# ROAM-Lab-ND/generalized_rbda

Measured on AMD Instinct MI355X. Metric: forward-dynamics evals/sec (batched random states), MIT Humanoid cluster model, higher is better.
Workload: dtype f32; 1 GPU; mit_humanoid.urdf cluster-ABA, 262144 random states per GPU; batch_per_gpu=262144, batch_global=262144, nq=25, nv=24, n_bodies=37, n_clusters=17, parallelism=batch-sharded x1, plan replicated

## Files before the change

### generalized_rbda_amd/csrc/capi.cpp

```cpp
#include <hip/hip_runtime.h>

#include <array>
#include <cassert>
#include <cmath>
#include <cstdio>
#include <cstdlib>
#include <cstring>
#include <map>
#include <memory>
#include <mutex>
#include <string>
#include <vector>

#include "../../include/grbda_hip.h"
#include "../../include/grbda_hip_vjp.h"
#include "../../include/grbda_model_desc.h"
#include "devplan.h"

namespace grbda_hip {
int urdf_to_blob(const char *const *paths, int n_paths, int ori_repr, std::vector<unsigned char> &blob,
                 std::string &err);

}

// ... 2471 lines not shown
        size_t B, int device, void *stream)
{
    if (!p) return set_err(GRBDA_EINVAL, "null plan");
    GRBDA_CALL_SCOPE(p);
    if (int rc = vjp_args<T>(p, q, qd, x, g, step, grad_q, grad_qd, grad_x, ydd_out, B)) return rc;
    if (B == 0) return GRBDA_OK;
    return vjp_run<T>(p, forward, q, qd, x, g, step, grad_q, grad_qd, grad_x, ydd_out, B, device, stream);
}
int vjp_host_f64(const grbda_plan *p, bool forward, const double *q, const double *qd, const double *x, const double *g, double step, double *grad_q,
                 double *grad_qd, double *grad_x, double *ydd_out, size_t B, int device)
{
    if (!p) return set_err(GRBDA_EINVAL, "null plan");
    GRBDA_CALL_SCOPE(p);
    if (int rc = vjp_args<double>(p, q, qd, x, g, step, grad_q, grad_qd, grad_x, ydd_out, B)) return rc;
    if (B == 0) return GRBDA_OK;
    const size_t nq = p->host.nq, nv = p->host.nv;
    DeviceTables *t = nullptr;
    if (int rc0 = ensure_device(p, device, &t)) return rc0;
    HostStage st;
    const double *bq = st.in(q, B * nq), *bqd = st.in(qd, B * nv), *bx = st.in(x, B * nv), *bg = st.in(g, B * nv);
    double *b1 = grad_q ? st.out(grad_q, B * nv) : nullptr, *b2 = grad_qd ? st.out(grad_qd, B * nv) : nullptr,
           *b3 = grad_x ? st.out(grad_x, B * nv) : nullptr, *b4 = ydd_out ? st.out(ydd_out, B * nv) : nullptr;
    return st.run([&] { return vjp_run<double>(p, forward, bq, bqd, bx, bg, step, b1, b2, b3, b4, B, device, nullptr); });
}

template <class T>
static std::string kernel_name_of(const grbda_plan *p, int kind, int n_cu, size_t B)
{
    const HostPlan &h = p->host;
    const char *tn = sizeof(T) == 4 ? "float" : "double";
    const char *alg = kind == 0 ? "aba" : "rnea";
    const Route r = kind == 0 ? choose_aba<T>(p, n_cu, B, false) : choose_rnea<T>(p, n_cu, B, false);
    char buf[160];
    const auto format = [&](const auto &cp, int gen1_waves) {
        const int segs = !cp.gens.empty() ? 2 : (!cp.diffs.empty() ? 1 : 0);
        if (r.path == ROUTE_GEN1)
            std::snprintf(buf, sizeof buf, "grbda_hip::%s_gen1_kernel<%s, %d, %s, %d>", alg, tn, cp.gens[0].n, cp.gens[0].kind ? "true" : "false", gen1_waves);
        else if (r.path == ROUTE_LM)
            std::snprintf(buf, sizeof buf, "grbda_hip::%s_chain_lm_kernel<%s, %d%s>", alg, tn, r.lm_waves, cp.diffs.empty() ? "" : ", true");
        else if (kind == 0)
            std::snprintf(buf, sizeof buf, "grbda_hip::aba_chain_kernel<%s, %d, %d>", tn, (sizeof(T) == 8 && !cp.gens.empty()) ? 1 : 2, segs);
        else
            std::snprintf(buf, sizeof buf, "grbda_hip::rnea_chain_kernel<%s, %d, %s>", tn, segs, cp.n_glb > 0 ? "true" : "false");
    };
    if (r.path == ROUTE_INTERPRETER) {
        bool loop = false;
        for (const ClusterRec &cr : h.lay64.clusters) loop = loop || cr.kind == CK_LOOP;
        std::snprintf(buf, sizeof buf, "grbda_hip::%s_kernel<%s, %s>", alg, tn, loop ? "true" : "false");
    } else if (kind == 0) {
        format(h.chain[r.slot], r.path == ROUTE_GEN1 ? gen1_waves_per_simd<T>(h.chain[r.slot].gens[0].n) : 0);
    } else {
        const RneaChainProgram &rp = h.rchain[r.slot == SLOT_F32_WIDE ? SLOT_F32 : r.slot];
        format(rp, r.path == ROUTE_GEN1 ? rnea_gen1_waves_per_simd<T>(rp.gens[0].n) : 0);
    }
    return buf;
}

template <class T>
int run_sharded(const grbda_plan *p, bool rnea, const T *q, const T *qd, const T *x, T *out, size_t B, int n_gpus)
{
    if (!p) return set_err(GRBDA_EINVAL, "null plan");
    GRBDA_CALL_SCOPE(p);
    if (!q || !qd || !x || !out) return set_err(GRBDA_EINVAL, "null argument");
    int count = 0;
    if (hipGetDeviceCount(&count) != hipSuccess || count <= 0)
        return set_err(GRBDA_ENODEVICE, "no HIP device available (there is no CPU fallback)");
    if (n_gpus < 1 || n_gpus > count) return set_err(GRBDA_EINVAL, "n_gpus out of range");
    if (B == 0) return GRBDA_OK;
    const size_t nq = p->host.nq, nv = p->host.nv;
    struct Shard {
        size_t b0 = 0, nb = 0;
        T *dq = nullptr, *dqd = nullptr, *dx = nullptr, *dout = nullptr;
        hipStream_t s = nullptr;
    };
    std::vector<Shard> sh(n_gpus);
    int rc = GRBDA_OK;
    hipError_t e = hipSuccess;
    for (int g = 0; g < n_gpus && rc == GRBDA_OK; g++) {
        Shard &S = sh[g];
        S.b0 = B * g / n_gpus;
        S.nb = B * (g + 1) / n_gpus - S.b0;
        if (S.nb == 0) continue;
        if ((e = hipSetDevice(g)) != hipSuccess || (e = hipStreamCreate(&S.s)) != hipSuccess ||
// ... 1106 lines not shown
```

### generalized_rbda_amd/csrc/chain_kernels.hip

```cpp
#include <hip/hip_runtime.h>

#include "devplan.h"

#ifndef GRBDA_CHAIN_UNIT
#define GRBDA_CHAIN_UNIT 0
#endif
#define GRBDA_KLDS (GRBDA_CHAIN_UNIT == 3)

namespace grbda_hip {

#include "devmath.h"

template <class T>
struct ChainTables {
    cptr<ChainSeg> segs;
    cptr<ChainLink> links;
    cptr<ChainPair> pairs;
    cptr<ChainFree> frees;
    cptr<ChainDiff> diffs;
    cptr<ChainGen> gens;
    cptr<ChainGenBody> gbodies;
    cptr<int32_t> cints;
    cptr<T> consts;
    int n_segs, nq, nv, ori_repr;
// ... 75 lines not shown
    {
        return *reinterpret_cast<const T *>(reinterpret_cast<const char *>(base_u + (size_t)(unsigned)(j * kWave)) + (size_t)lane_b);
    }
    __device__ __forceinline__ T q(int j) const { return row_ld(in_q_u, j); }
    __device__ __forceinline__ T qd(int j) const { return row_ld(in_qd_u, j); }
    __device__ __forceinline__ T x(int j) const { return row_ld(in_x_u, j); }
    int out_row;
    __device__ __forceinline__ T got(int j) const
    {
        return *reinterpret_cast<const T *>(reinterpret_cast<const char *>(out_u + (size_t)(unsigned)(j * kWave)) + (size_t)lane_b);
    }
    __device__ __forceinline__ void put_f(int j, T v) const
    {
        if constexpr (sizeof(T) == 4) {
            if (out_row >= 0) reinterpret_cast<T *>(grbda_smem)[(out_row + j) * kWave + lane] = v;
            else put(j, v);
        } else {
            out_f[j * kWave + lane] = v;
        }
    }
    T *out_f;
    __device__ __forceinline__ void set_out(int row)
    {
        out_row = row;
        out_f = row >= 0 ? reinterpret_cast<T *>(grbda_smem) + row * kWave : out_u;
    }
    __device__ __forceinline__ void put(int j, T v) const
    {
        *reinterpret_cast<T *>(reinterpret_cast<char *>(out_u + (size_t)(unsigned)(j * kWave)) + (size_t)lane_b) = v;
    }
};

template <class T>
__device__ __forceinline__ void vxz(const T (&v)[6], T qd, T (&c)[6])
{
    c[0] = v[1] * qd; c[1] = -v[0] * qd; c[2] = 0;
    c[3] = v[4] * qd; c[4] = -v[3] * qd; c[5] = 0;
}

template <class T, class I21>
__device__ __forceinline__ void bias_force(const I21 &I, const T (&v)[6], T (&p)[6])
{
    T Iv[6];
    symv_c(I, v, Iv);
    crf(v, Iv, p);
}

template <class T>
__device__ __forceinline__ void rotor_terms(cptr<T> Rp, const T (&vp)[6], T qdr, T (&tp)[6])
{
    T f[6], t[6];
#pragma unroll
    for (int j = 0; j < 6; j++) f[j] = Rp[j];
    crf(vp, f, t);
#pragma unroll
    for (int j = 0; j < 6; j++) tp[j] = qdr * t[j];
}
template <class T>
__device__ __forceinline__ void rotor_quad(cptr<T> Q, const T (&vp)[6], T (&tp)[6])
{
    T t[6];
    bias_force(Q, vp, t);
#pragma unroll
    for (int j = 0; j < 6; j++) tp[j] += t[j];
}

// ... 50 lines not shown
{
    if (perm < 0) {
        T E[9];
        rotate_z(s, c, C, E);
        xmotion(E, C + 9, vp, v);
        xmotion(E, C + 9, ap, a);
    } else if (perm == 0) {
        xmotion_p<T, 0>(s, c, C + 9, vp, v);
        xmotion_p<T, 0>(s, c, C + 9, ap, a);
    } else if (perm == 1) {
        xmotion_p<T, 1>(s, c, C + 9, vp, v);
        xmotion_p<T, 1>(s, c, C + 9, ap, a);
    } else {
        xmotion_p<T, 2>(s, c, C + 9, vp, v);
        xmotion_p<T, 2>(s, c, C + 9, ap, a);
    }
}
template <class T>
__device__ __forceinline__ void link_force_up(int perm, T s, T c, cptr<T> C, const T (&f)[6], T (&o)[6])
{
    if (perm < 0) {
        T E[9];
        rotate_z(s, c, C, E);
        xforce_inv(E, C + 9, f, o);
    } else if (perm == 0) {
        xforce_inv_p<T, 0>(s, c, C + 9, f, o);
    } else if (perm == 1) {
        xforce_inv_p<T, 1>(s, c, C + 9, f, o);
    } else {
        xforce_inv_p<T, 2>(s, c, C + 9, f, o);
    }
}

template <class T, bool SVG>
__device__ __forceinline__ void run_fwd(const ChainTables<T> &P, const ChainMem<T> &M, const ChainSeg &sg)
{
    T vp[6];
    {
        const ChainLink l0 = load_rec(P.links + sg.first);
        if (l0.lds_pv != -1) {
            if constexpr (SVG) M.acc_ld(l0.lds_pv, vp);
            else M.lds_ld(l0.lds_pv, vp);
        } else {
#pragma unroll
            for (int j = 0; j < 6; j++) vp[j] = 0;
        }
    }
    ChainLink l = load_rec(P.links + sg.first);
    T qi = M.q(l.q_index), qdi_in = M.qd(l.v_index);
    for (int i = 0; i < sg.count; i++) {
        const bool more = i + 1 < sg.count;
        const ChainLink ln = load_rec(P.links + (sg.first + (more ? i + 1 : i)));
        T qn = 0, qdn = 0;
        if (more) {
            qn = M.q(ln.q_index);
            qdn = M.qd(ln.v_index);
        }
        cptr<T> C = P.consts + l.cofs;
        const T g0 = C[kBodyConstFixed];
        T blk[8], v[6];
        const T ang = g0 * qi;
        sincos_t(ang, &blk[0], &blk[1]);
        link_down(perm_if<T>(kPermLink, l.perm), blk[0], blk[1], C, vp, v);
        v[2] += g0 * qdi_in;
#pragma unroll
        for (int j = 0; j < 6; j++) {
            blk[2 + j] = v[j];
            vp[j] = v[j];
        }
        if constexpr (SVG) M.acc_st(l.lds_sv, blk);
        else M.lds_st(l.lds_sv, blk);
        l = ln;
        qi = qn;
        qdi_in = qdn;
    }
}

constexpr int kChunk = 4;
template <class T>
__device__ __forceinline__ void run_fwd_c(const ChainTables<T> &P, const ChainMem<T> &M, const ChainSeg &sg)
{
    T vp[6];
    for (int base = 0; base < sg.count; base += kChunk) {
        const int n = sg.count - base;
        ChainLink L[kChunk];
        T qv[kChunk], qdv[kChunk];
#pragma unroll
        for (int u = 0; u < kChunk; u++) L[u] = load_rec(P.links + (sg.first + base + (u < n ? u : n - 1)));
#pragma unroll
        for (int u = 0; u < kChunk; u++) {
            qv[u] = M.q(L[u].q_index);
            qdv[u] = M.qd(L[u].v_index);
        }
        if (base == 0) {
            if (L[0].lds_pv != -1) {
                M.lds_ld(L[0].lds_pv, vp);
            } else {
#pragma unroll
                for (int j = 0; j < 6; j++) vp[j] = 0;
            }
        }
        T E[kChunk][9], r[kChunk][3], sc[kChunk][2], gq[kChunk];
#pragma unroll
        for (int u = 0; u < kChunk; u++) {
            if (u < n) {
                cptr<T> C = P.consts + L[u].cofs;
                const T g0 = C[kBodyConstFixed];
                sincos_t(g0 * qv[u], &sc[u][0], &sc[u][1]);
                rotate_z(sc[u][0], sc[u][1], C, E[u]);
#pragma unroll
                for (int j = 0; j < 3; j++) r[u][j] = C[9 + j];
                gq[u] = g0 * qdv[u];
            }
// ... 6 lines not shown
                v[2] += gq[u];
                blk[0] = sc[u][0];
                blk[1] = sc[u][1];
#pragma unroll
                for (int j = 0; j < 6; j++) {
                    blk[2 + j] = v[j];
                    vp[j] = v[j];
                }
                M.lds_st(L[u].lds_sv, blk);
            }
        }
    }
}

template <class T, int K>
__device__ __forceinline__ void xmotion_k(T s, T c, const T (&E)[9], cptr<T> C, const T (&m)[6], T (&o)[6])
{
    if constexpr (K < 0) xmotion(E, C + 9, m, o);
    else xmotion_p<T, K>(s, c, C + 9, m, o);
}
template <class T, int K>
__device__ __forceinline__ void xforce_inv_k(T s, T c, const T (&E)[9], cptr<T> C, const T (&f)[6], T (&o)[6])
{
    if constexpr (K < 0) xforce_inv(E, C + 9, f, o);
    else xforce_inv_p<T, K>(s, c, C + 9, f, o);
}
template <class T, int K, class A21>
__device__ __forceinline__ void congruence_k(T s, T c, const T (&E)[9], cptr<T> C, const A21 &A, T (&B)[21])
{
    if constexpr (K < 0) congruence(E, C + 9, A, B);
    else congruence_p<T, K>(s, c, C + 9, A, B);
}

template <class T, bool OSIM, int K1, int K2>
__device__ __forceinline__ void pair_bwd_k(const ChainTables<T> &P, const ChainMem<T> &M, const ChainPair &pr, T (&IA)[21],
                                           T (&psi)[6])
{
    cptr<T> C1 = P.consts + pr.cofs[0], C2 = P.consts + pr.cofs[1];
    T vp[6];
    M.acc_ld(pr.lds_pv, vp);
    const T y1 = M.q(pr.q_index), y2 = M.q(pr.q_index + 1);
    const T yd1 = M.qd(pr.v_index), yd2 = M.qd(pr.v_index + 1);
    T u[2] = {M.x(pr.v_index), M.x(pr.v_index + 1)};
    T D00 = 0, D01 = 0, D11 = 0;
    T F0[6], F1[6];

    T s1, c1, s2, c2, E1[9], E2[9], v1[6], v2[6], ch1[6], ch2[6];
    sincos_t(y1, &s1, &c1);
    if constexpr (K1 < 0) rotate_z(s1, c1, C1, E1);
    xmotion_k<T, K1>(s1, c1, E1, C1, vp, v1);
    v1[2] += yd1;
    vxz(v1, yd1, ch1);
    sincos_t(y2, &s2, &c2);
    if constexpr (K2 < 0) rotate_z(s2, c2, C2, E2);
    xmotion_k<T, K2>(s2, c2, E2, C2, v1, v2);
    v2[2] += yd2;
    vxz(v2, yd2, ch2);
    T ccl2[6];
    xmotion_k<T, K2>(s2, c2, E2, C2, ch1, ccl2);
#pragma unroll
    for (int j = 0; j < 6; j++) ccl2[j] += ch2[j];

    T IA1[21], psi1[6];
    {
        cptr<T> I2 = C2 + 12;
        T p2[6], h2[6];
        bias_force(I2, v2, p2);
#pragma unroll
// ... 48 lines not shown
        D11 += Rp[6] * gb * gb;
#pragma unroll
        for (int j = 0; j < 6; j++) {
            F0[j] += Rp[j] * ga;
            F1[j] += Rp[j] * gb;
            psi[j] += tp[j];
        }
    }
    const T r00 = rsqrt_t(D00), l10 = D01 * r00, r11 = rsqrt_t(D11 - l10 * l10);
    M.pivot(D00);
    M.pivot(D11 - l10 * l10);
    const T i00 = r00 * r00 + (l10 * r00 * r11) * (l10 * r00 * r11), i01 = -(l10 * r00) * r11 * r11, i11 = r11 * r11;
    T blk[14];
    auto solve2 = [&](T b0, T b1, T &x0, T &x1) {
        const T y0 = b0 * r00, y1 = (b1 - l10 * y0) * r11;
        x1 = y1 * r11;
        x0 = (y0 - l10 * x1) * r00;
    };
#pragma unroll
    for (int j = 0; j < 6; j++) solve2(F0[j], F1[j], blk[j], blk[6 + j]);
    solve2(u[0], u[1], blk[12], blk[13]);
    M.glb_st(pr.glb_k, blk);
    if constexpr (OSIM) {
        const T ex[7] = {i00, i01, i11, s1, c1, s2, c2};
        M.glb_st(pr.glb_k + 14, ex);
    }
#pragma unroll
    for (int r = 0; r < 6; r++) {
        psi[r] += F0[r] * blk[12] + F1[r] * blk[13];
#pragma unroll
        for (int cc = r; cc < 6; cc++) IA[sidx(r, cc)] -= F0[r] * blk[cc] + F1[r] * blk[6 + cc];
    }
}
template <class T, bool OSIM>
__device__ __forceinline__ void pair_bwd(const ChainTables<T> &P, const ChainMem<T> &M, const ChainPair &pr, T (&IA)[21],
                                         T (&psi)[6])
{
    if (perm_if<T>(kPermPair, pr.perm[0]) == 0 && pr.perm[1] == 0) pair_bwd_k<T, OSIM, 0, 0>(P, M, pr, IA, psi);
    else pair_bwd_k<T, OSIM, -1, -1>(P, M, pr, IA, psi);
}

template <class T>
__device__ __forceinline__ void pair_acc(const ChainTables<T> &P, const ChainMem<T> &M, const ChainPair &pr)
{
    T blk[14], va[12];
    M.glb_ld(pr.glb_k, blk);
    M.lds_ld(pr.lds_pva, va);
    T y0 = blk[12], y1 = blk[13];
#pragma unroll
    for (int j = 0; j < 6; j++) {
        y0 -= blk[j] * va[6 + j];
        y1 -= blk[6 + j] * va[6 + j];
    }
    M.put_f(pr.v_index, y0);
    M.put_f(pr.v_index + 1, y1);
}


template <class T, class TB>
__device__ __forceinline__ void diff_constraint(const TB &P, const ChainMem<T> &M, int tofs_i, int lds_w, const T (&qs)[4], T yd0,
                                                T yd1, T (&X)[4], T (&g)[2], T (&qdl)[2])
{
    cptr<int32_t> ip = P.cints + tofs_i;
    const int n_args = ip[0], n_atoms = ip[1];
    cptr<T> dp = P.consts + ip[2];
    for (int i = 0; i < n_args; i++) {
        cptr<T> w = dp + 5 * i;
        const T a = w[4] + w[0] * qs[0] + w[1] * qs[1] + w[2] * qs[2] + w[3] * qs[3];
// ... 349 lines not shown
        ydd0 -= blk[j] * ap[j];
        ydd1 -= blk[6 + j] * ap[j];
    }
    M.put_f(d.v_index, ydd0);
    M.put_f(d.v_index + 1, ydd1);
    if (d.lds_va >= 0) {
        cptr<T> C1 = P.consts + d.cofs[0], C2 = P.consts + d.cofs[1];
        const T yd0 = M.qd(d.v_index), yd1 = M.qd(d.v_index + 1);
        const T qd1 = blk[14] * yd0 + blk[15] * yd1, qd2 = blk[16] * yd0 + blk[17] * yd1;
        const T qdd1 = blk[14] * ydd0 + blk[15] * ydd1 + blk[18], qdd2 = blk[16] * ydd0 + blk[17] * ydd1 + blk[19];
        T E1[9], E2[9], v1[6], v2[6], a1[6], a2[6], c[6];
        const T sc[4] = {blk[20], blk[21], blk[22], blk[23]};
        diff_links(C1, C2, sc, vp, qd1, qd2, E1, E2, v1, v2);
        xmotion(E1, C1 + 9, ap, a1);
        vxz(v1, qd1, c);
#pragma unroll
        for (int j = 0; j < 6; j++) a1[j] += c[j];
        a1[2] += qdd1;
        xmotion(E2, C2 + 9, a1, a2);
        vxz(v2, qd2, c);
#pragma unroll
        for (int j = 0; j < 6; j++) a2[j] += c[j];
        a2[2] += qdd2;
        T out[12];
#pragma unroll
        for (int j = 0; j < 6; j++) {
            out[j] = v2[j];
            out[6 + j] = a2[j];
        }
        M.lds_st(d.lds_va, out);
    }
}

template <class T, bool OSIM, bool SVG, int ROT = 0>
__device__ __forceinline__ void run_bwd(const ChainTables<T> &P, const ChainMem<T> &M, const ChainSeg &sg)
{
    T IAc[21], psic[6];
    if (sg.head == HEAD_PAIR) {
        const ChainPair pr = load_rec(P.pairs + sg.head_arg);
        pair_bwd<T, OSIM>(P, M, pr, IAc, psic);
    } else if (sg.head == HEAD_SLOT) {
        T acc[27];
        M.acc_ld(sg.head_arg, acc);
#pragma unroll
        for (int j = 0; j < 21; j++) IAc[j] = acc[j];
#pragma unroll
        for (int j = 0; j < 6; j++) psic[j] = acc[21 + j];
    } else {
#pragma unroll
        for (int j = 0; j < 21; j++) IAc[j] = 0;
#pragma unroll
        for (int j = 0; j < 6; j++) psic[j] = 0;
    }
    ChainLink l = load_rec(P.links + sg.first);
    T yd = M.qd(l.v_index), tau_in = M.x(l.v_index), y_in = M.q(l.q_index);
    T blk[8];
    if constexpr (SVG) M.acc_ld(l.lds_sv, blk);
    for (int i = 0; i < sg.count; i++) {
        const bool more = i + 1 < sg.count;
        const ChainLink ln = load_rec(P.links + (sg.first + (more ? i + 1 : i)));
        T ydn = 0, taun = 0, yn = 0;
        if (more) {
            ydn = M.qd(ln.v_index);
            taun = M.x(ln.v_index);
            yn = M.q(ln.q_index);
        }
        T blkn[8];
        if constexpr (SVG) {
// ... 185 lines not shown
            T v[6], a[6], chat[6], sn, cs;
            sincos_t(g0 * yq, &sn, &cs);
            link_down2(perm_if<T>(kPermAcc, l.perm), sn, cs, C, vp, ap, v, a);
            v[2] += qdi;
            vxz(v, qdi, chat);
#pragma unroll
            for (int j = 0; j < 6; j++) a[j] += chat[j];
            a[2] += g0 * ydd;
            if (l.lds_va >= 0) {
                T va[12];
#pragma unroll
                for (int j = 0; j < 6; j++) {
                    va[j] = v[j];
                    va[6 + j] = a[j];
                }
                M.lds_st(l.lds_va, va);
            }
#pragma unroll
            for (int j = 0; j < 6; j++) {
                vp[j] = v[j];
                ap[j] = a[j];
            }
        }
        if (more) {
            l = ln;
            yd = ydn;
            yq = yqn;
#pragma unroll
            for (int j = 0; j < 7; j++) kb[j] = kn[j];
        }
    }
}

template <class T>
__device__ __forceinline__ void run_acc_c(const ChainTables<T> &P, const ChainMem<T> &M, const ChainSeg &sg)
{
    T vp[6], ap[6];
    for (int base = 0; base < sg.count; base += kChunk) {
        const int n = sg.count - base;
        ChainLink L[kChunk];
        T kb[kChunk][7], yd[kChunk], yq[kChunk];
#pragma unroll
        for (int u = 0; u < kChunk; u++) L[u] = load_rec(P.links + (sg.first + base + (u < n ? u : n - 1)));
#pragma unroll
        for (int u = 0; u < kChunk; u++) {
            yd[u] = M.qd(L[u].v_index);
            yq[u] = M.q(L[u].q_index);
        }
#pragma unroll
        for (int u = 0; u < kChunk; u++) M.glb_ld(L[u].glb_k, kb[u]);
        if (base == 0) {
            if (sg.lds_pva >= 0) {
                T va[12];
                M.lds_ld(sg.lds_pva, va);
#pragma unroll
                for (int j = 0; j < 6; j++) {
                    vp[j] = va[j];
                    ap[j] = va[6 + j];
                }
            } else {
#pragma unroll
                for (int j = 0; j < 6; j++) {
                    vp[j] = 0;
                    ap[j] = P.a_root[j];
                }
            }
        }
        T E[kChunk][9], r[kChunk][3], g0v[kChunk], qdi[kChunk];
// ... 18 lines not shown
                T ydd = kb[u][6];
#pragma unroll
                for (int rr = 0; rr < 6; rr++) ydd -= kb[u][rr] * ap[rr];
                M.put_f(l.v_index, ydd);
                if (l.has_child) {
                    T v[6], a[6], chat[6];
                    xmotion(E[u], r[u], vp, v);
                    xmotion(E[u], r[u], ap, a);
                    v[2] += qdi[u];
                    vxz(v, qdi[u], chat);
#pragma unroll
                    for (int j = 0; j < 6; j++) a[j] += chat[j];
                    a[2] += g0v[u] * ydd;
                    if (l.lds_va >= 0) {
                        T va[12];
#pragma unroll
                        for (int j = 0; j < 6; j++) {
                            va[j] = v[j];
                            va[6 + j] = a[j];
                        }
                        M.lds_st(l.lds_va, va);
                    }
#pragma unroll
                    for (int j = 0; j < 6; j++) {
                        vp[j] = v[j];
                        ap[j] = a[j];
                    }
                }
            }
        }
    }
}

template <class T>
__device__ __forceinline__ void free_fwd(const ChainTables<T> &P, const ChainMem<T> &M, const ChainFree &f)
{
    if (f.lds_v < 0) return;
    T v[6];
#pragma unroll
    for (int j = 0; j < 6; j++) v[j] = M.qd(f.v_index + j);
    M.lds_st(f.lds_v, v);
}

template <class T>
__device__ __forceinline__ void free_acc_inputs(const ChainTables<T> &P, const ChainMem<T> &M, const ChainFree &f, T (&o)[4], T (&r)[3]);
template <class T>
__device__ __forceinline__ void free_acc_core(const ChainTables<T> &P, const ChainMem<T> &M, const ChainFree &f, const T (&y0)[6],
                                              const T (&o)[4], const T (&r)[3], const T (&vb)[6]);
template <class T, bool OSIM>
__device__ __forceinline__ void free_bwd(const ChainTables<T> &P, const ChainMem<T> &M, const ChainFree &f, bool fuse_acc = false)
{
    cptr<T> Ic = P.consts + f.bofs;
    cptr<T> Ib = P.consts + f.iofs;
    T v[6], psi[6], IA[21];
#pragma unroll
    for (int j = 0; j < 6; j++) v[j] = M.qd(f.v_index + j);
    T o_[4] = {0, 0, 0, 0}, r_[3] = {0, 0, 0};
    if constexpr (!OSIM) {
        if (fuse_acc) free_acc_inputs(P, M, f, o_, r_);
    }
    bias_force(Ic, v, psi);
    if (f.lds_acc != -1) {
        T acc[27];
        M.acc_ld(f.lds_acc, acc);
#pragma unroll
        for (int j = 0; j < 21; j++) IA[j] = Ib[j] + acc[j];
#pragma unroll
        for (int j = 0; j < 6; j++) psi[j] += acc[21 + j];
        if (f.lds_acc2 != -1) {
            auto add = [&](int slot) {
                M.acc_ld(slot, acc);
#pragma unroll
                for (int j = 0; j < 21; j++) IA[j] += acc[j];
#pragma unroll
                for (int j = 0; j < 6; j++) psi[j] += acc[21 + j];
            };
            add(f.lds_acc2);
            if (f.lds_acc3 != -1) {
                add(f.lds_acc3);
                if (f.lds_acc4 != -1) add(f.lds_acc4);
            }
        }
    } else {
// ... 1 lines not shown
        for (int j = 0; j < 21; j++) IA[j] = Ib[j];
    }
    T D[6][6], u[6];
#pragma unroll
    for (int i = 0; i < 6; i++) {
        u[i] = M.x(f.v_index + i) - psi[i];
#pragma unroll
        for (int j = 0; j < 6; j++) D[i][j] = IA[sidx(i, j)];
    }
    Chol<T, 6> ch;
    ch.factor(D);
#pragma unroll
    for (int i = 0; i < 6; i++) M.pivot(ch.inv[i] < T(1e30) ? ch.inv[i] : T(0));
    ch.solve(u);
    if constexpr (!OSIM) {
        if (fuse_acc) {
            free_acc_core(P, M, f, u, o_, r_, v);
            return;
        }
    }
    M.glb_st(f.glb_y0, u);
    if constexpr (OSIM) {
        T ex[27];
#pragma unroll
        for (int i = 0; i < 6; i++) {
#pragma unroll
            for (int j = 0; j <= i; j++) ex[i * (i + 1) / 2 + j] = ch.L[i][j];
            ex[21 + i] = ch.inv[i];
        }
        M.glb_st(f.glb_y0 + 6, ex);
    }
}

template <class T>
__device__ __forceinline__ void free_acc_inputs(const ChainTables<T> &P, const ChainMem<T> &M, const ChainFree &f, T (&o)[4], T (&r)[3])
{
    const int nori = P.ori_repr == 0 ? 4 : 3;
#pragma unroll
    for (int j = 0; j < 4; j++) o[j] = j < nori ? M.q(f.q_index + 3 + j) : T(0);
#pragma unroll
    for (int j = 0; j < 3; j++) r[j] = M.q(f.q_index + j);
}
template <class T>
__device__ __forceinline__ void free_acc_core(const ChainTables<T> &P, const ChainMem<T> &M, const ChainFree &f, const T (&y0)[6],
                                              const T (&o)[4], const T (&r)[3], const T (&vb)[6])
{
    T E[9], g[6], ag[6];
    free_rotation(P.ori_repr, o, E);
#pragma unroll
    for (int j = 0; j < 6; j++) g[j] = P.a_root[j];
    xmotion(E, r, g, ag);
#pragma unroll
    for (int j = 0; j < 6; j++) M.put_f(f.v_index + j, y0[j] - ag[j]);
    if (f.lds_va >= 0) {
        T va[12];
#pragma unroll
        for (int j = 0; j < 6; j++) {
            va[j] = vb[j];
            va[6 + j] = y0[j];
        }
        M.lds_st(f.lds_va, va);
    }
}
template <class T>
__device__ __forceinline__ void free_acc(const ChainTables<T> &P, const ChainMem<T> &M, const ChainFree &f)
{
    T y0[6], o[4], r[3], vb[6];
    M.glb_ld(f.glb_y0, y0);
    free_acc_inputs(P, M, f, o, r);
#pragma unroll
    for (int j = 0; j < 6; j++) vb[j] = M.qd(f.v_index + j);
    free_acc_core(P, M, f, y0, o, r, vb);
}

#include "gen_segments.h"

#if GRBDA_CHAIN_UNIT == 2
template <class T>
struct ChainMemC : ChainMem<T> {
    int in_q, in_qd, in_x;
    T *out_g;
    __device__ __forceinline__ T q(int j) const { return reinterpret_cast<const T *>(grbda_smem)[(in_q + j) * kWave + this->lane]; }
    __device__ __forceinline__ T qd(int j) const { return reinterpret_cast<const T *>(grbda_smem)[(in_qd + j) * kWave + this->lane]; }
    __device__ __forceinline__ T x(int j) const { return reinterpret_cast<const T *>(grbda_smem)[(in_x + j) * kWave + this->lane]; }
    __device__ __forceinline__ void put(int j, T v) const
    {
        if (out_g) out_g[j] = v;
    }
    __device__ __forceinline__ void put_f(int j, T v) const { put(j, v); }
};

template <class T, int N, bool LOOP, class BODY>
__device__ __forceinline__ void gen1_tiles(int work_bytes, int nq, const T *__restrict__ q, const T *__restrict__ qd, const T *__restrict__ x,
                                           T *__restrict__ out, size_t B, unsigned long long *bad_count, BODY body)
{
    const int lane = threadIdx.x;
    ChainMemC<T> M;
    M.bad = 0;
// ... 83 lines not shown
template <class T>
int gen1_waves_per_simd(int n)
{
    return sizeof(T) == 4 ? (n <= 2 ? 3 : 2) : (n == 1 ? 2 : 1);
}
template int gen1_waves_per_simd<float>(int);
template int gen1_waves_per_simd<double>(int);
template <class T>
hipError_t launch_aba_gen1(const ChainDev<T> &P, int n, int implicit, const T *q, const T *qd, const T *tau, T *ydd, size_t B, int grid,
                           size_t lds_bytes, hipStream_t stream)
{
    if (implicit) {
        if (n == 1) return launch_gen1<T, 1, true>(P, q, qd, tau, ydd, B, grid, lds_bytes, stream);
        if (n == 2) return launch_gen1<T, 2, true>(P, q, qd, tau, ydd, B, grid, lds_bytes, stream);
        if (n == 3) return launch_gen1<T, 3, true>(P, q, qd, tau, ydd, B, grid, lds_bytes, stream);
        return launch_gen1<T, 4, true>(P, q, qd, tau, ydd, B, grid, lds_bytes, stream);
    }
    if (n == 1) return launch_gen1<T, 1, false>(P, q, qd, tau, ydd, B, grid, lds_bytes, stream);
    if (n == 2) return launch_gen1<T, 2, false>(P, q, qd, tau, ydd, B, grid, lds_bytes, stream);
    if (n == 3) return launch_gen1<T, 3, false>(P, q, qd, tau, ydd, B, grid, lds_bytes, stream);
    return launch_gen1<T, 4, false>(P, q, qd, tau, ydd, B, grid, lds_bytes, stream);
}
template hipError_t launch_aba_gen1<float>(const ChainDev<float> &, int, int, const float *, const float *, const float *, float *, size_t, int,
                                           size_t, hipStream_t);
template hipError_t launch_aba_gen1<double>(const ChainDev<double> &, int, int, const double *, const double *, const double *, double *,
                                            size_t, int, size_t, hipStream_t);
#endif

template <class T, int WPS, int MODE>
__global__ __launch_bounds__(kWave, WPS) void aba_chain_kernel(ChainDev<T> DP, const T *__restrict__ q, const T *__restrict__ qd,
                                                             const T *__restrict__ tau, T *__restrict__ ydd, size_t B,
                                                             T *__restrict__ scratch)
{
    constexpr bool DIFF = MODE >= 1, GEN = MODE == 2;
    ChainTables<T> P;
    P.segs = (cptr<ChainSeg>)DP.segs;
    P.links = (cptr<ChainLink>)DP.links;
    P.pairs = (cptr<ChainPair>)DP.pairs;
    P.frees = (cptr<ChainFree>)DP.frees;
    P.diffs = DIFF ? (cptr<ChainDiff>)DP.diffs : nullptr;
    P.gens = GEN ? (cptr<ChainGen>)DP.gens : nullptr;
    P.gbodies = GEN ? (cptr<ChainGenBody>)DP.gbodies : nullptr;
    P.cints = DIFF ? (cptr<int32_t>)DP.cints : nullptr;
    P.consts = (cptr<T>)DP.consts;
    P.n_segs = DP.n_segs;
    P.nq = DP.nq;
    P.nv = DP.nv;
    P.ori_repr = DP.ori_repr;
#pragma unroll
    for (int i = 0; i < 6; i++) P.a_root[i] = DP.a_root[i];
    const int lane = threadIdx.x;
    T *slab = scratch + (size_t)blockIdx.x * (size_t)(DP.n_glb_slots + P.nq + 2 * P.nv) * kWave;
    ChainMem<T> M;
    M.lane = lane;
    M.lane_b = (unsigned)lane * (unsigned)sizeof(T);
    M.gmul = 1;
    M.amask = ~0;
    M.glb_u = slab + (size_t)(P.nq + 2 * P.nv) * kWave;
    M.in_q_u = slab;
    M.in_qd_u = slab + (size_t)P.nq * kWave;
    M.in_x_u = slab + (size_t)(P.nq + P.nv) * kWave;
    M.out_u = slab + (size_t)(P.nq + P.nv) * kWave;
    M.set_out(DP.out_lds);
    M.bad = 0;

    const size_t n_tiles = (B + kWave - 1) / kWave;
    for (size_t tile = blockIdx.x; tile < n_tiles; tile += gridDim.x) {
        const size_t left = B - tile * kWave;
        const int rows_valid = left < (size_t)kWave ? (int)left : kWave;
        stage_inputs(q, qd, tau, tile, rows_valid, P.nq, P.nv, slab, lane, DP.lds_bytes);
        if (DP.fuse & 1) {
            const T *mine = reinterpret_cast<const T *>(grbda_smem) + (kWave * P.nq + lane * P.nv + DP.stage_v_index);
            T v[6];
#pragma unroll
            for (int j = 0; j < 6; j++) v[j] = mine[j];
            wave_lds_fence();
            M.lds_st(DP.stage_lds_v, v);
        }
        for (int s = 0; s < P.n_segs; s++) {
            const ChainSeg sg = load_rec(P.segs + s);
            switch (sg.op) {
                case SEG_RUN_FWD:
                    if (DP.sv_global) run_fwd<T, true>(P, M, sg);
                    else run_fwd_c(P, M, sg);
                    break;
                case SEG_RUN_BWD: {
                    if (DP.sv_global) run_bwd<T, false, true>(P, M, sg);
                    else if (sg.rot_kind == 1) run_bwd<T, false, false, 1>(P, M, sg);
                    else run_bwd<T, false, false>(P, M, sg);
                    break;
                }
                case SEG_RUN_ACC:
                    run_acc_c(P, M, sg);
                    break;
                case SEG_PAIR_ACC: pair_acc(P, M, load_rec(P.pairs + sg.first)); break;
                case SEG_FREE_FWD:
                    if (!((DP.fuse & 1) && s == 0)) free_fwd(P, M, load_rec(P.frees + sg.first));
                    break;
                case SEG_FREE_BWD: free_bwd<T, false>(P, M, load_rec(P.frees + sg.first), (DP.fuse & 2) != 0); break;
                case SEG_DIFF_FWD:
                    if constexpr (DIFF) diff_fwd(P, M, load_rec(P.diffs + sg.first));
                    break;
                case SEG_DIFF_BWD:
// ... 553 lines not shown
        asm volatile("s_waitcnt vmcnt(0)" ::: "memory");
    }
}

template <class T>
hipError_t launch_osim_chain(const ChainDev<T> &P, const OsimArgs<T> &A, const T *q, const T *zeros, T *Linv, T *J, size_t B,
                             T *scratch, int grid, size_t lds_bytes, hipStream_t stream)
{
    hipLaunchKernelGGL((osim_chain_kernel<T>), dim3(grid), dim3(kWave), lds_bytes, stream, P, A, q, zeros, Linv, J, B, scratch);
    return hipGetLastError();
}
#if GRBDA_CHAIN_UNIT == 0
template hipError_t launch_osim_chain<float>(const ChainDev<float> &, const OsimArgs<float> &, const float *, const float *, float *,
                                             float *, size_t, float *, int, size_t, hipStream_t);
template hipError_t launch_osim_chain<double>(const ChainDev<double> &, const OsimArgs<double> &, const double *, const double *,
                                              double *, double *, size_t, double *, int, size_t, hipStream_t);
#endif

hipError_t launch_aba_chain_diff_f64(const ChainDev<double> &P, const double *q, const double *qd, const double *tau, double *ydd, size_t B,
                                     double *scratch, int grid, size_t lds_bytes, hipStream_t stream);
template <class T>
hipError_t launch_aba_chain_gen(const ChainDev<T> &P, const T *q, const T *qd, const T *tau, T *ydd, size_t B, T *scratch, int grid,
                                size_t lds_bytes, hipStream_t stream);
template <class T>
hipError_t launch_aba_chain(const ChainDev<T> &P, const T *q, const T *qd, const T *tau, T *ydd, size_t B, T *scratch, int grid,
                            size_t lds_bytes, hipStream_t stream)
{
    if (P.n_gens > 0) return launch_aba_chain_gen<T>(P, q, qd, tau, ydd, B, scratch, grid, lds_bytes, stream);
    if (P.n_diffs > 0) {
        if constexpr (sizeof(T) == 8) {
            return launch_aba_chain_diff_f64(P, q, qd, tau, ydd, B, scratch, grid, lds_bytes, stream);
        } else {
            hipLaunchKernelGGL((aba_chain_kernel<T, 2, 1>), dim3(grid), dim3(kWave), lds_bytes, stream, P, q, qd, tau, ydd, B, scratch);
            return hipGetLastError();
        }
    }
    hipLaunchKernelGGL((aba_chain_kernel<T, 2, 0>), dim3(grid), dim3(kWave), lds_bytes, stream, P, q, qd, tau, ydd, B, scratch);
    return hipGetLastError();
}
#if GRBDA_CHAIN_UNIT == 0
template hipError_t launch_aba_chain<float>(const ChainDev<float> &, const float *, const float *, const float *, float *, size_t,
                                            float *, int, size_t, hipStream_t);
template hipError_t launch_aba_chain<double>(const ChainDev<double> &, const double *, const double *, const double *, double *,
                                             size_t, double *, int, size_t, hipStream_t);
#elif GRBDA_CHAIN_UNIT == 1
hipError_t launch_aba_chain_diff_f64(const ChainDev<double> &P, const double *q, const double *qd, const double *tau, double *ydd, size_t B,
                                     double *scratch, int grid, size_t lds_bytes, hipStream_t stream)
{
    hipLaunchKernelGGL((aba_chain_kernel<double, 2, 1>), dim3(grid), dim3(kWave), lds_bytes, stream, P, q, qd, tau, ydd, B, scratch);
    return hipGetLastError();
}
#elif GRBDA_CHAIN_UNIT == 2
template <class T>
hipError_t launch_aba_chain_gen(const ChainDev<T> &P, const T *q, const T *qd, const T *tau, T *ydd, size_t B, T *scratch, int grid,
                                size_t lds_bytes, hipStream_t stream)
{
    if constexpr (sizeof(T) == 8)
        hipLaunchKernelGGL((aba_chain_kernel<T, 1, 2>), dim3(grid), dim3(kWave), lds_bytes, stream, P, q, qd, tau, ydd, B, scratch);
    else
        hipLaunchKernelGGL((aba_chain_kernel<T, 2, 2>), dim3(grid), dim3(kWave), lds_bytes, stream, P, q, qd, tau, ydd, B, scratch);
    return hipGetLastError();
}
template hipError_t launch_aba_chain_gen<float>(const ChainDev<float> &, const float *, const float *, const float *, float *, size_t,
                                                float *, int, size_t, hipStream_t);
template hipError_t launch_aba_chain_gen<double>(const ChainDev<double> &, const double *, const double *, const double *, double *,
                                                 size_t, double *, int, size_t, hipStream_t);
// ... 671 lines not shown
{
    const bool glb = P.n_glb_slots > 0;
    if (P.n_gens > 0) return launch_rnea_chain_gen<T>(P, q, qd, ydd, tau, B, scratch, grid, lds_bytes, stream);
    if (P.n_diffs > 0 && glb) hipLaunchKernelGGL((rnea_chain_kernel<T, 1, true>), dim3(grid), dim3(kWave), lds_bytes, stream, P, q, qd, ydd, tau, B, scratch);
    else if (P.n_diffs > 0) hipLaunchKernelGGL((rnea_chain_kernel<T, 1, false>), dim3(grid), dim3(kWave), lds_bytes, stream, P, q, qd, ydd, tau, B, scratch);
    else if (glb) hipLaunchKernelGGL((rnea_chain_kernel<T, 0, true>), dim3(grid), dim3(kWave), lds_bytes, stream, P, q, qd, ydd, tau, B, scratch);
    else hipLaunchKernelGGL((rnea_chain_kernel<T, 0, false>), dim3(grid), dim3(kWave), lds_bytes, stream, P, q, qd, ydd, tau, B, scratch);
    return hipGetLastError();
}
#if GRBDA_CHAIN_UNIT == 0
template hipError_t launch_rnea_chain<float>(const RneaChainDev<float> &, const float *, const float *, const float *, float *, size_t,
                                             float *, int, size_t, hipStream_t);
template hipError_t launch_rnea_chain<double>(const RneaChainDev<double> &, const double *, const double *, const double *, double *,
                                              size_t, double *, int, size_t, hipStream_t);
#endif


static hipError_t set_max_dynamic_lds(const void *const *kernels, int n)
{
    for (int i = 0; i < n; i++) {
        const hipError_t e = hipFuncSetAttribute(kernels[i], hipFuncAttributeMaxDynamicSharedMemorySize, 160 * 1024);
        if (e != hipSuccess) return e;
    }
    return hipSuccess;
}
hipError_t set_max_dynamic_lds_chain_unit1();
hipError_t set_max_dynamic_lds_chain_unit2();
hipError_t set_max_dynamic_lds_chain_unit3();
#if GRBDA_CHAIN_UNIT == 0
hipError_t set_max_dynamic_lds_chain()
{
    const void *const kernels[] = {
        reinterpret_cast<const void *>(&aba_chain_kernel<float, 2, 0>), reinterpret_cast<const void *>(&aba_chain_kernel<float, 2, 1>),
        reinterpret_cast<const void *>(&aba_chain_kernel<double, 2, 0>),
        reinterpret_cast<const void *>(&rnea_chain_kernel<float, 0, false>), reinterpret_cast<const void *>(&rnea_chain_kernel<float, 1, false>),
        reinterpret_cast<const void *>(&rnea_chain_kernel<double, 0, false>), reinterpret_cast<const void *>(&rnea_chain_kernel<double, 1, false>),
        reinterpret_cast<const void *>(&rnea_chain_kernel<float, 0, true>), reinterpret_cast<const void *>(&rnea_chain_kernel<float, 1, true>),
        reinterpret_cast<const void *>(&rnea_chain_kernel<double, 0, true>), reinterpret_cast<const void *>(&rnea_chain_kernel<double, 1, true>),
        reinterpret_cast<const void *>(&osim_chain_kernel<float>), reinterpret_cast<const void *>(&osim_chain_kernel<double>)};
    const hipError_t e = set_max_dynamic_lds(kernels, static_cast<int>(sizeof(kernels) / sizeof(kernels[0])));
    if (e != hipSuccess) return e;
    const hipError_t e1 = set_max_dynamic_lds_chain_unit1();
    if (e1 != hipSuccess) return e1;
    const hipError_t e2 = set_max_dynamic_lds_chain_unit2();
    return e2 != hipSuccess ? e2 : set_max_dynamic_lds_chain_unit3();
}
#elif GRBDA_CHAIN_UNIT == 1
hipError_t set_max_dynamic_lds_chain_unit1()
{
    const void *const kernels[] = {reinterpret_cast<const void *>(&aba_chain_kernel<double, 2, 1>),
                                   reinterpret_cast<const void *>(&aba_chain_lm_kernel<double, 2>)};
    return set_max_dynamic_lds(kernels, 2);
}
#elif GRBDA_CHAIN_UNIT == 3
hipError_t set_max_dynamic_lds_chain_unit3()
{
    const void *const kernels[] = {reinterpret_cast<const void *>(&aba_chain_lm_kernel<float, 2>), reinterpret_cast<const void *>(&aba_chain_lm_kernel<float, 4>),
                                   reinterpret_cast<const void *>(&aba_chain_lm_kernel<float, 2, true>), reinterpret_cast<const void *>(&aba_chain_lm_kernel<float, 4, true>),
                                   reinterpret_cast<const void *>(&aba_chain_lm_kernel<double, 4>),
                                   reinterpret_cast<const void *>(&rnea_chain_lm_kernel<float, 2>), reinterpret_cast<const void *>(&rnea_chain_lm_kernel<float, 4>),
                                   reinterpret_cast<const void *>(&rnea_chain_lm_kernel<double, 2>), reinterpret_cast<const void *>(&rnea_chain_lm_kernel<double, 4>),
                                   reinterpret_cast<const void *>(&rnea_chain_lm_kernel<float, 2, true>), reinterpret_cast<const void *>(&rnea_chain_lm_kernel<float, 4, true>)};
    return set_max_dynamic_lds(kernels, 11);
}
#else
hipError_t set_max_dynamic_lds_chain_unit2()
// ... 13 lines not shown
```

### generalized_rbda_amd/csrc/devmath.h

```cpp
#pragma once

template <class U>
using cptr = const U __attribute__((address_space(4))) *;

template <class U>
__device__ __forceinline__ U load_rec(cptr<U> p)
{
    static_assert(sizeof(U) % 4 == 0, "plan records are arrays of int32");
    U out;
    cptr<int32_t> src = (cptr<int32_t>)p;
    int32_t *dst = reinterpret_cast<int32_t *>(&out);
#pragma unroll
    for (int i = 0; i < (int)(sizeof(U) / 4); i++) dst[i] = src[i];
    return out;
}

extern __shared__ __attribute__((aligned(16))) unsigned char grbda_smem[];

__host__ __device__ constexpr int sidx(int i, int j)
{
    return i <= j ? (i * 6 - i * (i - 1) / 2 + (j - i)) : (j * 6 - j * (j - 1) / 2 + (i - j));
}

template <class T>
// ... 346 lines not shown
                                             size_t tile, int rows_valid, int nq, int nv, T *slab, int lane,
                                             int lds_bytes)
{
    const unsigned bq = (unsigned)(kWave * nq) * (unsigned)sizeof(T), bv = (unsigned)(kWave * nv) * (unsigned)sizeof(T);
    if ((int)(bq + 2 * bv) <= lds_bytes) {
        stage_issue(q, tile, rows_valid, nq, 0u, lane);
        stage_issue(qd, tile, rows_valid, nv, bq, lane);
        stage_issue(x, tile, rows_valid, nv, bq + bv, lane);
        asm volatile("s_waitcnt vmcnt(0)" ::: "memory");
        wave_lds_fence();
        stage_transpose(nq, 0u, slab, lane);
        stage_transpose(nv, bq, slab + (size_t)nq * kWave, lane);
        stage_transpose(nv, bq + bv, slab + (size_t)(nq + nv) * kWave, lane);
        wave_lds_fence();
    } else {
        stage_issue(q, tile, rows_valid, nq, 0u, lane);
        asm volatile("s_waitcnt vmcnt(0)" ::: "memory");
        wave_lds_fence();
        stage_transpose(nq, 0u, slab, lane);
        wave_lds_fence();
        stage_issue(qd, tile, rows_valid, nv, 0u, lane);
        asm volatile("s_waitcnt vmcnt(0)" ::: "memory");
        wave_lds_fence();
        stage_transpose(nv, 0u, slab + (size_t)nq * kWave, lane);
        wave_lds_fence();
        stage_issue(x, tile, rows_valid, nv, 0u, lane);
        asm volatile("s_waitcnt vmcnt(0)" ::: "memory");
        wave_lds_fence();
        stage_transpose(nv, 0u, slab + (size_t)(nq + nv) * kWave, lane);
        wave_lds_fence();
    }
}

template <class T>
__device__ __forceinline__ void write_outputs(const T *rows, T *__restrict__ out, size_t tile, int rows_valid, int nv,
                                              int lane)
{
    asm volatile("s_waitcnt vmcnt(0) lgkmcnt(0)" ::: "memory");
    T *stage = reinterpret_cast<T *>(grbda_smem);
    constexpr int V = 16 / (int)sizeof(T);
    if ((nv % V) == 0) {
        struct alignas(16) Vec { T v[V]; };
        Vec *mine = reinterpret_cast<Vec *>(stage + lane * nv);
        for (int c = 0; c < nv; c += V) {
            Vec x;
#pragma unroll
            for (int k = 0; k < V; k++) x.v[k] = rows[(size_t)(c + k) * kWave + lane];
            mine[c / V] = x;
        }
    } else {
        for (int c = 0; c < nv; c++) stage[lane * nv + c] = rows[(size_t)c * kWave + lane];
    }
    wave_lds_fence();
    T *dst = out + tile * (size_t)kWave * (size_t)nv;
    const int total = rows_valid * nv;
    for (int i = 0; i < nv; i++) {
        const int j = i * kWave + lane;
        if (j < total) dst[j] = stage[j];
    }
    wave_lds_fence();
}

template <class T>
__device__ __forceinline__ void write_outputs_lds(int out_row, T *__restrict__ out, size_t tile, int rows_valid, int nv, int lane)
{
    asm volatile("s_waitcnt lgkmcnt(0)" ::: "memory");
// ... 181 lines not shown
```

### generalized_rbda_amd/csrc/devplan.h

```cpp
#pragma once
#include <cstdlib>
#include <hip/hip_runtime.h>

#include "plan.h"

namespace grbda_hip {

inline size_t lds_workgroups_per_cu(size_t lds_bytes)
{
    if (lds_bytes == 0) return 32;
    constexpr size_t granule = 1280;
    return (160u * 1024u) / ((lds_bytes + granule - 1) / granule * granule);
}


template <class T>
struct DevPlan {
    const Step *steps;
    int n_steps;
    const ClusterRec *clusters;
    const BodyRec *bodies;
    const T *consts;
    const int32_t *cints;
    const int32_t *acc_k;
// ... 36 lines not shown
                            int32_t *ok, int ok_and, size_t B, int max_iter, T tol, T *scratch, int grid, size_t lds_bytes, hipStream_t stream);
template <class T>
hipError_t launch_poses(const DevPlan<T> &P, int n_clusters, const T *q, T *Xa, size_t B, int grid, hipStream_t stream);
template <class T>
hipError_t launch_twists(const DevPlan<T> &P, int n_clusters, int n_span, const T *q, const T *qd_span, const T *qdd_span, T *V, size_t B,
                         int grid, hipStream_t stream);
hipError_t set_max_dynamic_lds();

template <class T>
struct ChainDev {
    const ChainSeg *segs;
    const ChainLink *links;
    const ChainPair *pairs;
    const ChainFree *frees;
    const ChainDiff *diffs;
    int n_diffs;
    const ChainGen *gens;
    const ChainGenBody *gbodies;
    int n_gens;
    const int32_t *cints;
    const T *consts;
    int n_segs;
    int nq, nv;
    int n_glb_slots;
    int lds_bytes;
    int ori_repr;
    int debug;
    int sv_global;
    int out_lds;
    int fuse, stage_lds_v, stage_v_index;
    unsigned long long *bad_count;
    T a_root[6];
};
template <class T>
hipError_t launch_aba_chain(const ChainDev<T> &P, const T *q, const T *qd, const T *tau, T *ydd, size_t B, T *scratch, int grid,
                            size_t lds_bytes, hipStream_t stream);
template <class T>
hipError_t launch_aba_chain_lm(const ChainDev<T> &P, const T *q, const T *qd, const T *tau, T *ydd, size_t B, T *scratch, int grid,
                               size_t lds_bytes, hipStream_t stream, int n_waves);
hipError_t set_max_dynamic_lds_chain();
template <class T>
hipError_t launch_aba_gen1(const ChainDev<T> &P, int n, int implicit, const T *q, const T *qd, const T *tau, T *ydd, size_t B, int grid,
                           size_t lds_bytes, hipStream_t stream);
template <class T>
int gen1_waves_per_simd(int n);

template <class T>
struct RneaChainDev {
    const RneaSeg *segs;
    const RneaLink *links;
    const RneaPair *pairs;
    const RneaFree *frees;
    const RneaDiff *diffs;
    int n_diffs;
    const ChainGen *gens;
    const ChainGenBody *gbodies;
    int n_gens;
    const int32_t *cints;
    const T *consts;
    int n_segs;
    int nq, nv;
    int n_glb_slots;
    int lds_bytes;
    int ori_repr;
    T a_root[6];
};
// ... 165 lines not shown
```

Baseline: 2.046 billion evals/s.

## Hold per-lane q, qd, tau inputs in registers for f32 chain ABA kernel

Adds an in-register input mode for the f32 chain ABA kernel. Inputs are staged through LDS once and then loaded into per-lane 32-wide vector registers instead of being transposed into an LDS slab. Index accesses like M.q(j) then read from registers. This removes repeated LDS reads and the transpose, at the cost of about 96 extra VGPRs per lane, which can lower occupancy or cause spills. It also adds dynamic indexing into vector registers, which may compile to scratch or waterfall code.

Result: faster. 2.271 billion evals/s (median of 6 runs) (+11.0%).

```diff
diff --git a/generalized_rbda_amd/csrc/capi.cpp b/generalized_rbda_amd/csrc/capi.cpp
--- a/generalized_rbda_amd/csrc/capi.cpp
+++ b/generalized_rbda_amd/csrc/capi.cpp
@@ -2527,14 +2527,15 @@
     const char *alg = kind == 0 ? "aba" : "rnea";
     const Route r = kind == 0 ? choose_aba<T>(p, n_cu, B, false) : choose_rnea<T>(p, n_cu, B, false);
     char buf[160];
-    const auto format = [&](const auto &cp, int gen1_waves) {
+    const auto format = [&](const auto &cp, int gen1_waves, bool inreg = false) {
         const int segs = !cp.gens.empty() ? 2 : (!cp.diffs.empty() ? 1 : 0);
         if (r.path == ROUTE_GEN1)
             std::snprintf(buf, sizeof buf, "grbda_hip::%s_gen1_kernel<%s, %d, %s, %d>", alg, tn, cp.gens[0].n, cp.gens[0].kind ? "true" : "false", gen1_waves);
         else if (r.path == ROUTE_LM)
             std::snprintf(buf, sizeof buf, "grbda_hip::%s_chain_lm_kernel<%s, %d%s>", alg, tn, r.lm_waves, cp.diffs.empty() ? "" : ", true");
         else if (kind == 0)
-            std::snprintf(buf, sizeof buf, "grbda_hip::aba_chain_kernel<%s, %d, %d>", tn, (sizeof(T) == 8 && !cp.gens.empty()) ? 1 : 2, segs);
+            std::snprintf(buf, sizeof buf, "grbda_hip::aba_chain_kernel<%s, %d, %d>", tn, (sizeof(T) == 8 && !cp.gens.empty()) ? 1 : 2,
+                          inreg ? kModeInReg : segs);
         else
             std::snprintf(buf, sizeof buf, "grbda_hip::rnea_chain_kernel<%s, %d, %s>", tn, segs, cp.n_glb > 0 ? "true" : "false");
     };
@@ -2543,7 +2544,9 @@
         for (const ClusterRec &cr : h.lay64.clusters) loop = loop || cr.kind == CK_LOOP;
         std::snprintf(buf, sizeof buf, "grbda_hip::%s_kernel<%s, %s>", alg, tn, loop ? "true" : "false");
     } else if (kind == 0) {
-        format(h.chain[r.slot], r.path == ROUTE_GEN1 ? gen1_waves_per_simd<T>(h.chain[r.slot].gens[0].n) : 0);
+        const ChainProgram &cp = h.chain[r.slot];
+        format(cp, r.path == ROUTE_GEN1 ? gen1_waves_per_simd<T>(cp.gens[0].n) : 0,
+               chain_inputs_in_registers(sizeof(T), static_cast<int>(cp.gens.size()), static_cast<int>(cp.diffs.size()), cp.sv_global ? 1 : 0, h.nq, h.nv));
     } else {
         const RneaChainProgram &rp = h.rchain[r.slot == SLOT_F32_WIDE ? SLOT_F32 : r.slot];
         format(rp, r.path == ROUTE_GEN1 ? rnea_gen1_waves_per_simd<T>(rp.gens[0].n) : 0);
diff --git a/generalized_rbda_amd/csrc/chain_kernels.hip b/generalized_rbda_amd/csrc/chain_kernels.hip
--- a/generalized_rbda_amd/csrc/chain_kernels.hip
+++ b/generalized_rbda_amd/csrc/chain_kernels.hip
@@ -131,6 +131,15 @@
 };
 
 template <class T>
+struct ChainMemR : ChainMem<T> {
+    typedef T Row __attribute__((ext_vector_type(kInRegCols)));
+    Row rq, rqd, rx;
+    __device__ __forceinline__ T q(int j) const { return rq[j]; }
+    __device__ __forceinline__ T qd(int j) const { return rqd[j]; }
+    __device__ __forceinline__ T x(int j) const { return rx[j]; }
+};
+
+template <class T>
 __device__ __forceinline__ void vxz(const T (&v)[6], T qd, T (&c)[6])
 {
     c[0] = v[1] * qd; c[1] = -v[0] * qd; c[2] = 0;
@@ -247,8 +256,8 @@
     }
 }
 
-template <class T, bool SVG>
-__device__ __forceinline__ void run_fwd(const ChainTables<T> &P, const ChainMem<T> &M, const ChainSeg &sg)
+template <class T, bool SVG, class MM>
+__device__ __forceinline__ void run_fwd(const ChainTables<T> &P, const MM &M, const ChainSeg &sg)
 {
     T vp[6];
     {
@@ -292,8 +301,8 @@
 }
 
 constexpr int kChunk = 4;
-template <class T>
-__device__ __forceinline__ void run_fwd_c(const ChainTables<T> &P, const ChainMem<T> &M, const ChainSeg &sg)
+template <class T, class MM>
+__device__ __forceinline__ void run_fwd_c(const ChainTables<T> &P, const MM &M, const ChainSeg &sg)
 {
     T vp[6];
     for (int base = 0; base < sg.count; base += kChunk) {
@@ -366,8 +375,8 @@
     else congruence_p<T, K>(s, c, C + 9, A, B);
 }
 
-template <class T, bool OSIM, int K1, int K2>
-__device__ __forceinline__ void pair_bwd_k(const ChainTables<T> &P, const ChainMem<T> &M, const ChainPair &pr, T (&IA)[21],
+template <class T, bool OSIM, int K1, int K2, class MM>
+__device__ __forceinline__ void pair_bwd_k(const ChainTables<T> &P, const MM &M, const ChainPair &pr, T (&IA)[21],
                                            T (&psi)[6])
 {
     cptr<T> C1 = P.consts + pr.cofs[0], C2 = P.consts + pr.cofs[1];
@@ -482,8 +491,8 @@
         for (int cc = r; cc < 6; cc++) IA[sidx(r, cc)] -= F0[r] * blk[cc] + F1[r] * blk[6 + cc];
     }
 }
-template <class T, bool OSIM>
-__device__ __forceinline__ void pair_bwd(const ChainTables<T> &P, const ChainMem<T> &M, const ChainPair &pr, T (&IA)[21],
+template <class T, bool OSIM, class MM>
+__device__ __forceinline__ void pair_bwd(const ChainTables<T> &P, const MM &M, const ChainPair &pr, T (&IA)[21],
                                          T (&psi)[6])
 {
     if (perm_if<T>(kPermPair, pr.perm[0]) == 0 && pr.perm[1] == 0) pair_bwd_k<T, OSIM, 0, 0>(P, M, pr, IA, psi);
@@ -899,8 +908,8 @@
     }
 }
 
-template <class T, bool OSIM, bool SVG, int ROT = 0>
-__device__ __forceinline__ void run_bwd(const ChainTables<T> &P, const ChainMem<T> &M, const ChainSeg &sg)
+template <class T, bool OSIM, bool SVG, int ROT = 0, class MM>
+__device__ __forceinline__ void run_bwd(const ChainTables<T> &P, const MM &M, const ChainSeg &sg)
 {
     T IAc[21], psic[6];
     if (sg.head == HEAD_PAIR) {
@@ -1152,8 +1161,8 @@
     }
 }
 
-template <class T>
-__device__ __forceinline__ void run_acc_c(const ChainTables<T> &P, const ChainMem<T> &M, const ChainSeg &sg)
+template <class T, class MM>
+__device__ __forceinline__ void run_acc_c(const ChainTables<T> &P, const MM &M, const ChainSeg &sg)
 {
     T vp[6], ap[6];
     for (int base = 0; base < sg.count; base += kChunk) {
@@ -1238,8 +1247,8 @@
     }
 }
 
-template <class T>
-__device__ __forceinline__ void free_fwd(const ChainTables<T> &P, const ChainMem<T> &M, const ChainFree &f)
+template <class T, class MM>
+__device__ __forceinline__ void free_fwd(const ChainTables<T> &P, const MM &M, const ChainFree &f)
 {
     if (f.lds_v < 0) return;
     T v[6];
@@ -1248,13 +1257,13 @@
     M.lds_st(f.lds_v, v);
 }
 
-template <class T>
-__device__ __forceinline__ void free_acc_inputs(const ChainTables<T> &P, const ChainMem<T> &M, const ChainFree &f, T (&o)[4], T (&r)[3]);
+template <class T, class MM>
+__device__ __forceinline__ void free_acc_inputs(const ChainTables<T> &P, const MM &M, const ChainFree &f, T (&o)[4], T (&r)[3]);
 template <class T>
 __device__ __forceinline__ void free_acc_core(const ChainTables<T> &P, const ChainMem<T> &M, const ChainFree &f, const T (&y0)[6],
                                               const T (&o)[4], const T (&r)[3], const T (&vb)[6]);
-template <class T, bool OSIM>
-__device__ __forceinline__ void free_bwd(const ChainTables<T> &P, const ChainMem<T> &M, const ChainFree &f, bool fuse_acc = false)
+template <class T, bool OSIM, class MM>
+__device__ __forceinline__ void free_bwd(const ChainTables<T> &P, const MM &M, const ChainFree &f, bool fuse_acc = false)
 {
     cptr<T> Ic = P.consts + f.bofs;
     cptr<T> Ib = P.consts + f.iofs;
@@ -1322,8 +1331,8 @@
     }
 }
 
-template <class T>
-__device__ __forceinline__ void free_acc_inputs(const ChainTables<T> &P, const ChainMem<T> &M, const ChainFree &f, T (&o)[4], T (&r)[3])
+template <class T, class MM>
+__device__ __forceinline__ void free_acc_inputs(const ChainTables<T> &P, const MM &M, const ChainFree &f, T (&o)[4], T (&r)[3])
 {
     const int nori = P.ori_repr == 0 ? 4 : 3;
 #pragma unroll
@@ -1352,8 +1361,8 @@
         M.lds_st(f.lds_va, va);
     }
 }
-template <class T>
-__device__ __forceinline__ void free_acc(const ChainTables<T> &P, const ChainMem<T> &M, const ChainFree &f)
+template <class T, class MM>
+__device__ __forceinline__ void free_acc(const ChainTables<T> &P, const MM &M, const ChainFree &f)
 {
     T y0[6], o[4], r[3], vb[6];
     M.glb_ld(f.glb_y0, y0);
@@ -1503,7 +1512,7 @@
                                                              const T *__restrict__ tau, T *__restrict__ ydd, size_t B,
                                                              T *__restrict__ scratch)
 {
-    constexpr bool DIFF = MODE >= 1, GEN = MODE == 2;
+    constexpr bool DIFF = MODE == 1 || MODE == 2, GEN = MODE == 2, INREG = MODE == kModeInReg;
     ChainTables<T> P;
     P.segs = (cptr<ChainSeg>)DP.segs;
     P.links = (cptr<ChainLink>)DP.links;
@@ -1522,7 +1531,7 @@
     for (int i = 0; i < 6; i++) P.a_root[i] = DP.a_root[i];
     const int lane = threadIdx.x;
     T *slab = scratch + (size_t)blockIdx.x * (size_t)(DP.n_glb_slots + P.nq + 2 * P.nv) * kWave;
-    ChainMem<T> M;
+    std::conditional_t<INREG, ChainMemR<T>, ChainMem<T>> M;
     M.lane = lane;
     M.lane_b = (unsigned)lane * (unsigned)sizeof(T);
     M.gmul = 1;
@@ -1539,7 +1548,8 @@
     for (size_t tile = blockIdx.x; tile < n_tiles; tile += gridDim.x) {
         const size_t left = B - tile * kWave;
         const int rows_valid = left < (size_t)kWave ? (int)left : kWave;
-        stage_inputs(q, qd, tau, tile, rows_valid, P.nq, P.nv, slab, lane, DP.lds_bytes);
+        if constexpr (INREG) stage_inputs_reg<kInRegCols>(q, qd, tau, tile, rows_valid, P.nq, P.nv, M.rq, M.rqd, M.rx, lane, DP.lds_bytes);
+        else stage_inputs(q, qd, tau, tile, rows_valid, P.nq, P.nv, slab, lane, DP.lds_bytes);
         if (DP.fuse & 1) {
             const T *mine = reinterpret_cast<const T *>(grbda_smem) + (kWave * P.nq + lane * P.nv + DP.stage_v_index);
             T v[6];
@@ -2159,6 +2169,12 @@
             return launch_aba_chain_diff_f64(P, q, qd, tau, ydd, B, scratch, grid, lds_bytes, stream);
         } else {
             hipLaunchKernelGGL((aba_chain_kernel<T, 2, 1>), dim3(grid), dim3(kWave), lds_bytes, stream, P, q, qd, tau, ydd, B, scratch);
+            return hipGetLastError();
+        }
+    }
+    if constexpr (sizeof(T) == 4) {
+        if (chain_inputs_in_registers(sizeof(T), P.n_gens, P.n_diffs, P.sv_global, P.nq, P.nv)) {
+            hipLaunchKernelGGL((aba_chain_kernel<T, 2, kModeInReg>), dim3(grid), dim3(kWave), lds_bytes, stream, P, q, qd, tau, ydd, B, scratch);
             return hipGetLastError();
         }
     }
@@ -2896,6 +2912,7 @@
 {
     const void *const kernels[] = {
         reinterpret_cast<const void *>(&aba_chain_kernel<float, 2, 0>), reinterpret_cast<const void *>(&aba_chain_kernel<float, 2, 1>),
+        reinterpret_cast<const void *>(&aba_chain_kernel<float, 2, kModeInReg>),
         reinterpret_cast<const void *>(&aba_chain_kernel<double, 2, 0>),
         reinterpret_cast<const void *>(&rnea_chain_kernel<float, 0, false>), reinterpret_cast<const void *>(&rnea_chain_kernel<float, 1, false>),
         reinterpret_cast<const void *>(&rnea_chain_kernel<double, 0, false>), reinterpret_cast<const void *>(&rnea_chain_kernel<double, 1, false>),
diff --git a/generalized_rbda_amd/csrc/devmath.h b/generalized_rbda_amd/csrc/devmath.h
--- a/generalized_rbda_amd/csrc/devmath.h
+++ b/generalized_rbda_amd/csrc/devmath.h
@@ -402,6 +402,63 @@
     }
 }
 
+template <class T, int N, class ROW>
+__device__ __forceinline__ void stage_row_regs(int ncols, unsigned lds_byte_off, ROW &r, int lane)
+{
+    const T *stage = reinterpret_cast<const T *>(grbda_smem + lds_byte_off);
+    constexpr int V = 16 / (int)sizeof(T);
+    static_assert(N % V == 0, "whole 16-byte reads");
+    if ((ncols % V) == 0 && (lds_byte_off % 16u) == 0) {
+        struct alignas(16) Vec { T v[V]; };
+        const Vec *rows = reinterpret_cast<const Vec *>(stage + lane * ncols);
+#pragma unroll
+        for (int c = 0; c < N; c += V) {
+            if (c < ncols) {
+                const Vec x = rows[c / V];
+#pragma unroll
+                for (int k = 0; k < V; k++) r[c + k] = x.v[k];
+            }
+        }
+        return;
+    }
+#pragma unroll
+    for (int c = 0; c < N; c++)
+        if (c < ncols) r[c] = stage[lane * ncols + c];
+}
+template <int N, class T, class ROW>
+__device__ __forceinline__ void stage_inputs_reg(const T *__restrict__ q, const T *__restrict__ qd, const T *__restrict__ x, size_t tile,
+                                                 int rows_valid, int nq, int nv, ROW &rq, ROW &rqd, ROW &rx, int lane, int lds_bytes)
+{
+    const unsigned bq = (unsigned)(kWave * nq) * (unsigned)sizeof(T), bv = (unsigned)(kWave * nv) * (unsigned)sizeof(T);
+    if ((int)(bq + 2 * bv) <= lds_bytes) {
+        stage_issue(q, tile, rows_valid, nq, 0u, lane);
+        stage_issue(qd, tile, rows_valid, nv, bq, lane);
+        stage_issue(x, tile, rows_valid, nv, bq + bv, lane);
+        asm volatile("s_waitcnt vmcnt(0)" ::: "memory");
+        wave_lds_fence();
+        stage_row_regs<T, N>(nq, 0u, rq, lane);
+        stage_row_regs<T, N>(nv, bq, rqd, lane);
+        stage_row_regs<T, N>(nv, bq + bv, rx, lane);
+        wave_lds_fence();
+    } else {
+        stage_issue(q, tile, rows_valid, nq, 0u, lane);
+        asm volatile("s_waitcnt vmcnt(0)" ::: "memory");
+        wave_lds_fence();
+        stage_row_regs<T, N>(nq, 0u, rq, lane);
+        wave_lds_fence();
+        stage_issue(qd, tile, rows_valid, nv, 0u, lane);
+        asm volatile("s_waitcnt vmcnt(0)" ::: "memory");
+        wave_lds_fence();
+        stage_row_regs<T, N>(nv, 0u, rqd, lane);
+        wave_lds_fence();
+        stage_issue(x, tile, rows_valid, nv, 0u, lane);
+        asm volatile("s_waitcnt vmcnt(0)" ::: "memory");
+        wave_lds_fence();
+        stage_row_regs<T, N>(nv, 0u, rx, lane);
+        wave_lds_fence();
+    }
+}
+
 template <class T>
 __device__ __forceinline__ void write_outputs(const T *rows, T *__restrict__ out, size_t tile, int rows_valid, int nv,
                                               int lane)
diff --git a/generalized_rbda_amd/csrc/devplan.h b/generalized_rbda_amd/csrc/devplan.h
--- a/generalized_rbda_amd/csrc/devplan.h
+++ b/generalized_rbda_amd/csrc/devplan.h
@@ -92,6 +92,12 @@
     unsigned long long *bad_count;
     T a_root[6];
 };
+constexpr int kInRegCols = 32;
+constexpr int kModeInReg = 3;
+inline bool chain_inputs_in_registers(size_t elem, int n_gens, int n_diffs, int sv_global, int nq, int nv)
+{
+    return elem == 4 && n_gens == 0 && n_diffs == 0 && !sv_global && nq <= kInRegCols && nv <= kInRegCols;
+}
 template <class T>
 hipError_t launch_aba_chain(const ChainDev<T> &P, const T *q, const T *qd, const T *tau, T *ydd, size_t B, T *scratch, int grid,
                             size_t lds_bytes, hipStream_t stream);
```
